# BaratiLab/MeshDQN

Measured on AMD Instinct MI355X. Metric: env steps/sec (ys930 ~2k-tri), higher is better.
Workload: dtype f64; 1 GPU; ys930 (876 vertices / 1570 triangles), 128 envs per GPU, S3 env step (remesh+smooth+interp+forces+state+1 IPCS step+Q-fwd); mesh=ys930, envs_per_gpu=128, parallelism=dp1 (independent envs sharded, no data-path collective)

## Files before the change

### meshdqn_amd/csrc/mdq_smooth_linear.hip

```cpp
#include <hip/hip_runtime.h>

#include <cstdlib>

#include "../../include/meshdqn_hip.h"
#include "mdq_internal.h"

namespace mdq_smooth_lin {
constexpr int LNV = 1024;
constexpr int LNT = 2048;
#ifndef MDQ_SMOOTH_LWG
#define MDQ_SMOOTH_LWG 768
#endif
constexpr int LWG = MDQ_SMOOTH_LWG;
constexpr int SCT = 512;
constexpr int TRW = LWG / 64 < 11 ? LWG / 64 : 11;
static_assert(LWG == 512 || LWG == 768, "workgroup shape");
constexpr int BS = 32;
constexpr int NSLOT = 14;
constexpr int NNARROW = 4;
constexpr int MAXNB = 16;
constexpr int MAXLOW = 8;
constexpr int SROW = 32;
constexpr int ZOFF = LNV * 16;
constexpr int PBUF = (LNV + 1) * 16;
// ... 274 lines not shown
  const double* mgs = reinterpret_cast<const double*>(mg);
  unsigned char* cur = lds + OFF_CUR;
  double* G = reinterpret_cast<double*>(lds + OFF_G);
  const int* ptr = reinterpret_cast<const int*>(lds + OFF_PTR);
  for (int b = 0; b < nb; ++b) {
    const u4 meta = *reinterpret_cast<const u4*>(lds + OFF_SROW + (b * BS + i) * SROW + h * 16);
    d2 M[8];
    load_m(M, mg, b, i, h);
    const d2 v0 = *reinterpret_cast<const d2*>(cur + (meta.x & 0xFFFF)), v1 = *reinterpret_cast<const d2*>(cur + (meta.x >> 16));
    const d2 v2 = *reinterpret_cast<const d2*>(cur + (meta.y & 0xFFFF)), v3 = *reinterpret_cast<const d2*>(cur + (meta.y >> 16));
    const d2 v4 = *reinterpret_cast<const d2*>(cur + (meta.z & 0xFFFF)), v5 = *reinterpret_cast<const d2*>(cur + (meta.z >> 16));
    const d2 v6 = *reinterpret_cast<const d2*>(cur + (meta.w & 0xFFFF));
    const double gx = halves_sum(((v0.x + v1.x) + (v2.x + v3.x)) + ((v4.x + v5.x) + v6.x));
    const double gy = halves_sum(((v0.y + v1.y) + (v2.y + v3.y)) + ((v4.y + v5.y) + v6.y));
    if (h == 0) {
      G[i] = gx;
      G[BS + i] = gy;
    }
    asm volatile("" ::: "memory");
    const d2* gqx = reinterpret_cast<const d2*>(G + 16 * h);
    const d2* gqy = reinterpret_cast<const d2*>(G + BS + 16 * h);
    double ax0 = 0.0, ax1 = 0.0, ay0 = 0.0, ay1 = 0.0;
#pragma unroll
    for (int t = 0; t < 8; ++t) {
      const d2 ggx = gqx[t], ggy = gqy[t];
      ax0 = __builtin_fma(M[t].x, ggx.x, ax0);
      ax1 = __builtin_fma(M[t].y, ggx.y, ax1);
      ay0 = __builtin_fma(M[t].x, ggy.x, ay0);
      ay1 = __builtin_fma(M[t].y, ggy.y, ay1);
    }
    const double xx = halves_sum(ax0 + ax1), xy = halves_sum(ay0 + ay1);
    const int soff = meta.w >> 16;
    if (h == 0) *reinterpret_cast<d2*>(cur + soff) = d2{xx, xy};
    asm volatile("" ::: "memory");
    unsigned long long fm = __builtin_amdgcn_ballot_w64(h == 0 && fixv[soff >> 4] != 0);
    while (fm) {
      const int r = __ffsll((long long)fm) - 1;
      fm &= fm - 1;
      const int v = __builtin_amdgcn_readlane(soff, r) >> 4;
      const d2 xs = exact_vertex(lds, v, l, OLD);
      const d2 xt = *reinterpret_cast<const d2*>(cur + v * 16);
      const double kk = (double)(ptr[v + 1] - ptr[v]);
      const double ddx = (xs.x - xt.x) * kk, ddy = (xs.y - xt.y) * kk;
      const double mjr = mgs[(((size_t)(b * 2 + (r >> 4)) * 8 + ((r & 15) >> 1)) * 32 + i) * 2 + (r & 1)];
      if (h == 0 && i >= r) {
        d2 xc = *reinterpret_cast<const d2*>(cur + soff);
        xc.x = __builtin_fma(mjr, ddx, xc.x);
        xc.y = __builtin_fma(mjr, ddy, xc.y);
        if (i == r) xc = xs;
        *reinterpret_cast<d2*>(cur + soff) = xc;
      }
      asm volatile("" ::: "memory");
    }
  }
}

__device__ __forceinline__ void sequential_sweep(unsigned char* lds, int n_int, int lane) {
  const uint16_t* ivert = reinterpret_cast<const uint16_t*>(lds + OFF_IVERT);
  unsigned char* cur = lds + OFF_CUR;
  for (int r = 0; r < n_int; ++r) {
    const int v = ivert[r];
    const d2 xs = exact_vertex(lds, v, lane & 7, cur);
    if (lane == 0) *reinterpret_cast<d2*>(cur + v * 16) = xs;
    asm volatile("" ::: "memory");
  }
}

#ifdef MDQ_LIN_TRACE
__device__ long long mdq_lin_trace_buf[16];
#define LT_STAMP(k) { __syncthreads(); const long long tn_ = __builtin_amdgcn_s_memtime(); if (threadIdx.x == 0 && blockIdx.x == 0) mdq_lin_trace_buf[k] += tn_ - tq_; tq_ = tn_; }
extern "C" int mdq_lin_trace_host(long long* out, int reset) {
  if (hipMemcpyFromSymbol(out, HIP_SYMBOL(mdq_lin_trace_buf), sizeof(long long) * 16) != hipSuccess) return -1;
  if (reset) { long long z[16] = {0}; if (hipMemcpyToSymbol(HIP_SYMBOL(mdq_lin_trace_buf), z, sizeof z) != hipSuccess) return -1; }
  return 0;
}
#else
#define LT_STAMP(k)
#endif

__global__ __launch_bounds__(LWG) void smooth_linear_kernel(int NV, int NT, double* coords, const int32_t* cells,
                                                            const int32_t* nv_, const int32_t* nt_, const int32_t* iters_,
                                                            const int32_t* rem, const int32_t* rstat, int iters_env,
                                                            double* mws, int64_t mstride, int32_t* redo, int32_t* stats,
                                                            int gather_all) {
  __shared__ __attribute__((aligned(16))) unsigned char lds[LDS_BYTES];
  const int b = blockIdx.x, tid = threadIdx.x, lane = tid & 63, wave = tid >> 6;
  const int S = iters_ ? iters_[b] : ((rem[b] >= 0 && rstat[b] == 0) ? iters_env : 0);
  if (S <= 0) {
    if (tid == 0) redo[b] = stats[3 * b] = stats[3 * b + 1] = stats[3 * b + 2] = 0;
    return;
  }
  const int nv = nv_[b], nt = nt_[b];
  double2* x = reinterpret_cast<double2*>(coords) + (int64_t)b * NV;
  const int32_t* tri = cells + (int64_t)b * NT * 3;
  int* ptr = reinterpret_cast<int*>(lds + OFF_PTR);
  uint32_t* inc = reinterpret_cast<uint32_t*>(lds + OFF_INC);
  uint16_t* rk = reinterpret_cast<uint16_t*>(lds + OFF_RK);
  uint16_t* ivert = reinterpret_cast<uint16_t*>(lds + OFF_IVERT);
  unsigned char* lmeta = lds + OFF_LMETA;
  uint16_t* kdeg = reinterpret_cast<uint16_t*>(lds + OFF_KDEG);
  int* misc = reinterpret_cast<int*>(lds + OFF_MISC);
  int* part = reinterpret_cast<int*>(lds + OFF_PART);
  uint32_t* tmp = reinterpret_cast<uint32_t*>(lds + OFF_TMP);
  uint16_t* nbl = reinterpret_cast<uint16_t*>(lds + OFF_NB);
  int* cnt = reinterpret_cast<int*>(lds + OFF_SROW + 3 * LNT * 4);
  static_assert(3 * LNT * 4 + LNV * 4 <= LNV * SROW, "cnt scratch");
#ifdef MDQ_LIN_TRACE
  long long tq_ = __builtin_amdgcn_s_memtime();
#endif
  for (int v = tid; v < LNV; v += LWG) cnt[v] = 0;
  if (tid < 4) misc[tid] = tid == 2 ? 1 : tid == 3 && gather_all ? -1 : 0;
  if (tid < 32) reinterpret_cast<double*>(lds + OFF_R2K)[tid] = tid ? 1.0 / (2.0 * tid) : 0.0;
  __syncthreads();
  for (int t = tid; t < nt; t += LWG)
    for (int k = 0; k < 3; ++k) atomicAdd(&cnt[tri[3 * t + k]], 1);
  __syncthreads();
  scan_inclusive(cnt, part);
  for (int v = tid; v < LNV; v += LWG) ptr[v + 1] = cnt[v];
  if (tid == 0) ptr[0] = 0;
  __syncthreads();
  for (int v = tid; v < LNV; v += LWG) cnt[v] = 0;
  __syncthreads();
  for (int t = tid; t < nt; t += LWG) {
    const int vs[3] = {tri[3 * t], tri[3 * t + 1], tri[3 * t + 2]};
    for (int k = 0; k < 3; ++k) {
      const int v = vs[k], a = vs[(k + 1) % 3], c = vs[(k + 2) % 3];
      const int q = ptr[v] + atomicAdd(&cnt[v], 1);
      tmp[q] = (uint32_t)a | ((uint32_t)c << 10) | ((uint32_t)t << 20);
    }
  }
  __syncthreads();
  LT_STAMP(0)
  for (int v = tid; v < LNV; v += LWG) {
    const int q0 = ptr[v], k = ptr[v + 1] - q0;
    bool interior = v < nv && k > 0 && k <= MAXNB;
    if (v < nv && k > MAXNB) misc[2] = 0;
    int nn = 0;
    if (interior) {
      if (k <= 8) {
        uint32_t ent[8];
#pragma unroll
        for (int j = 0; j < 8; ++j) ent[j] = j < k ? tmp[q0 + j] : 0xFFFFFFFFu;
#pragma unroll
        for (int e = 0; e < 8; ++e) {
          int rank = 0;
#pragma unroll
          for (int j = 0; j < 8; ++j) rank += ent[j] < ent[e];
          if (e < k) inc[q0 + rank] = ent[e];
        }
      } else {
        for (int e = 0; e < k; ++e) {
          const uint32_t my = tmp[q0 + e];
          int rank = 0;
          for (int j = 0; j < k; ++j) rank += (tmp[q0 + j] >> 20) < (my >> 20);
          inc[q0 + rank] = my;
        }
      }
      for (int e = 0; e < k; ++e) {
        const uint32_t w = inc[q0 + e];
        for (int s = 0; s < 2; ++s) {
          const uint32_t id = s ? (w >> 10) & 0x3FF : w & 0x3FF;
          int f = -1;
          for (int j = 0; j < nn; ++j)
            if ((nbl[v * MAXNB + j] & 0x3FF) == id) f = j;
          if (f >= 0) {
            nbl[v * MAXNB + f] += 1 << 10;
          } else if (nn < MAXNB) {
            nbl[v * MAXNB + nn++] = (uint16_t)(id | (1 << 10));
          } else {
            interior = false;
          }
        }
      }
      for (int j = 0; j < nn; ++j) interior = interior && (nbl[v * MAXNB + j] >> 10) == 2;
      interior = interior && nn == k;
    }
    cnt[v] = interior ? 1 : 0;
  }
  __syncthreads();
  LT_STAMP(1)
  scan_inclusive(cnt, part);
  const int n_int = cnt[LNV - 1];
  const int nb = (n_int + BS - 1) / BS;
  __syncthreads();
  for (int v = tid; v < LNV; v += LWG) {
    const bool interior = cnt[v] != (v ? cnt[v - 1] : 0);
    rk[v] = interior ? (uint16_t)(cnt[v] - 1) : (uint16_t)0xFFFF;
    if (interior) ivert[cnt[v] - 1] = (uint16_t)v;
  }
  __syncthreads();
  for (int v = tid; v < nv; v += LWG)
    if (rk[v] == 0xFFFF)
      for (int q = ptr[v]; q < ptr[v + 1]; ++q) inc[q] = 0xFFFFFFFFu;
  LT_STAMP(2)
  for (int r = tid; r < nb * BS; r += LWG) {
    uint16_t slots[16];
#pragma unroll
    for (int s = 0; s < 16; ++s) slots[s] = (uint16_t)ZOFF;
    int ns = 0, nl = 0, k = 1;
    if (r < n_int) {
      const int v = ivert[r], q0 = ptr[v];
      k = ptr[v + 1] - q0;
      for (int j = 0; j < k; ++j) {
        const int w = nbl[v * MAXNB + j] & 0x3FF;
        const int rw = rk[w];
        if (rw != 0xFFFF && w < v && (rw >> 5) == (r >> 5)) {
          if (nl < MAXLOW) lmeta[r * MAXLOW + nl] = (unsigned char)(rw & 31);
          ++nl;
        } else {
          if (ns < NSLOT) {
            const int pos = (ns & 1) * 8 + (ns >> 1);
#pragma unroll
            for (int s = 0; s < 16; ++s)
              if (s == pos) slots[s] = (uint16_t)(w * 16);
          }
          ++ns;
        }
      }
      if (ns > NSLOT || nl > MAXLOW) misc[2] = 0;
      if (ns > 2 * NNARROW) atomicOr(&misc[3], 1 << (r >> 5));
      slots[7] = (uint16_t)(v * 16);
      for (int q = q0; q < q0 + k; ++q) {
        const uint32_t w = inc[q];
        const int a = w & 0x3FF, c = (w >> 10) & 0x3FF;
        inc[q] = (w & 0xFFFFF) | ((uint32_t)v << 20) | ((uint32_t)(rk[a] != 0xFFFF && a < v) << 30) |
                 ((uint32_t)(rk[c] != 0xFFFF && c < v) << 31);
      }
    }
    kdeg[r] = (uint16_t)(k | (min(nl, MAXLOW) << 8));
    uint32_t wds[8];
#pragma unroll
    for (int s = 0; s < 8; ++s) wds[s] = (uint32_t)slots[2 * s] | ((uint32_t)slots[2 * s + 1] << 16);
    *reinterpret_cast<u4*>(lds + OFF_SROW + r * SROW) = u4{wds[0], wds[1], wds[2], wds[3]};
    *reinterpret_cast<u4*>(lds + OFF_SROW + r * SROW + 16) = u4{wds[4], wds[5], wds[6], wds[7]};
  }
  __syncthreads();
  LT_STAMP(3)
  const bool eligible = misc[2] != 0 && n_int > 0;
  if (!eligible) {
    static_assert(mdq_smoothing::LDS_BYTES <= LDS_BYTES && mdq_smoothing::SNV == LNV && mdq_smoothing::SNT == LNT, "hand-back in place");
    __syncthreads();
    mdq_smoothing::smooth_env(lds, b, NV, NT, coords, cells, nv_, nt_, S, nullptr);
    if (tid == 0) {
      redo[b] = S;
      stats[3 * b] = stats[3 * b + 1] = stats[3 * b + 2] = 0;
    }
    return;
  }
  double* mg = mws + (int64_t)b * mstride;
  {
    double* T = reinterpret_cast<double*>(lds + OFF_TRI) + wave * 528;
    const double* r2ktab = reinterpret_cast<const double*>(lds + OFF_R2K);
    for (int blk = wave < TRW ? wave : nb; blk < nb; blk += TRW) {
      const int r0 = blk * BS, j = lane & 31;
      const uint32_t kdv = kdeg[r0 + j];
      const uint2 lmv = *reinterpret_cast<const uint2*>(lmeta + (r0 + j) * MAXLOW);
      if (lane < 32) {
        for (int i = 0; i < BS; ++i) {
          const uint32_t kd = (uint32_t)__builtin_amdgcn_readlane((int)kdv, i);
          const uint32_t lo = (uint32_t)__builtin_amdgcn_readlane((int)lmv.x, i), hi = (uint32_t)__builtin_amdgcn_readlane((int)lmv.y, i);
          const int nl = kd >> 8;
          double val = 0.0;
          for (int t = 0; t < nl; ++t) {
            const int w = (int)(((t < 4 ? lo : hi) >> (8 * (t & 3))) & 0xFFu);
            if (j <= w) val += T[w * (w + 1) / 2 + j];
          }
          val = val * (2.0 * r2ktab[kd & 0xFF]) + (i == j ? 1.0 : 0.0);
          if (j <= i) T[i * (i + 1) / 2 + j] = val;
          asm volatile("" ::: "memory");
        }
      }
      asm volatile("s_waitcnt lgkmcnt(0)" ::: "memory");
      const int i = lane & 31, h = lane >> 5;
      d2* out = reinterpret_cast<d2*>(mg) + ((size_t)(blk * 2 + h) * 8) * 32 + i;
      d2* out01 = reinterpret_cast<d2*>(lds + OFF_M01) + ((blk * 2 + h) * 8) * 32 + i;
      for (int t = 0; t < 8; ++t) {
        const int j0 = 16 * h + 2 * t;
        const double m0 = j0 <= i ? T[i * (i + 1) / 2 + j0] * (2.0 * r2ktab[kdeg[r0 + j0] & 0xFF]) : 0.0;
        const double m1 = j0 + 1 <= i ? T[i * (i + 1) / 2 + j0 + 1] * (2.0 * r2ktab[kdeg[r0 + j0 + 1] & 0xFF]) : 0.0;
        out[t * 32] = d2{m0, m1};
        if (blk < 2) out01[t * 32] = d2{m0, m1};
      }
      asm volatile("s_waitcnt lgkmcnt(0)" ::: "memory");
    }
  }
  __threadfence_block();
  __syncthreads();
  LT_STAMP(4)
  for (int v = tid; v <= LNV; v += LWG) {
    d2 p = {0.0, 0.0};
    if (v < nv) {
      const double2 xv = x[v];
      p = d2{xv.x, xv.y};
    }
    *reinterpret_cast<d2*>(lds + OFF_CUR + v * 16) = p;
    *reinterpret_cast<d2*>(lds + OFF_SNAP + v * 16) = p;
    *reinterpret_cast<d2*>(lds + OFF_SNAP + PBUF + v * 16) = p;
  }
  __syncthreads();
  LT_STAMP(5)
  const d2* mgd = reinterpret_cast<const d2*>(mg);
  constexpr int NVAL = 2 * (LWG / 256);
  const int vw = (wave & 3) >= 2 ? 2 * (wave >> 2) + (wave & 1) : -1;
  const int ne = 3 * nt, npass = (ne + 63) / 64;
  unsigned char* fixv = lds + OFF_FIXV;
  auto copy_pos = [&](int dst_off, int src_off) {
    for (int v = tid; v < nv; v += LWG)
      *reinterpret_cast<d2*>(lds + dst_off + v * 16) = *reinterpret_cast<const d2*>(lds + src_off + v * 16);
  };
  auto solve_fast = [&]() {
    if (wave == 0) {
      __builtin_amdgcn_s_setprio(3);
      solve_sweep<0>(lds, mgd, nb, lane);
      __builtin_amdgcn_s_setprio(0);
    } else if (wave == 1) {
      __builtin_amdgcn_s_setprio(3);
      solve_sweep<1>(lds, mgd, nb, lane);
      __builtin_amdgcn_s_setprio(0);
    }
  };
  int s = 0, n_repaired = 0, n_rounds = 0, n_sentback = 0, n_seq = 0;
  bool checked = true, pending = false;
  while (true) {
    if (s >= S && !pending) break;
    if (checked) {
      const int snap = OFF_SNAP + (s & 1) * PBUF;
      for (int v = tid; v < LNV + 16; v += LWG) fixv[v] = 0;
      int rounds = 0, nflag = 0;
      while (true) {
        __syncthreads();
        if (nflag == 0) {
          solve_fast();
        } else if (wave == 0) {
          repair_sweep(lds, mgd, nb, lane, lds + snap);
        }
        if (tid == 0) misc[1] = 0;
        __syncthreads();
        bool bad = false;
        for (int p = wave; p < npass; p += LWG / 64) bad |= validate_entry<true>(lds, 64 * p + lane, ne, lds + snap, lds + OFF_CUR);
        if (bad) misc[1] = 1;
        __syncthreads();
        if (!misc[1]) break;
        nflag = 1;
        ++n_rounds;
        copy_pos(OFF_CUR, snap);
        if (++rounds >= MAXROUNDS) {
          __syncthreads();
          if (wave == 0) sequential_sweep(lds, n_int, lane);
          __syncthreads();
          ++n_seq;
          break;
        }
      }
      copy_pos(OFF_SNAP + ((s + 1) & 1) * PBUF, OFF_CUR);
      __syncthreads();
      ++s;
      if (rounds == 0) {
        checked = false;
        pending = false;
      } else {
        ++n_repaired;
      }
    } else {
      if (s < S) solve_fast();
      bool bad = false;
      if (pending) {
        const unsigned char* OLD = lds + OFF_SNAP + ((s - 1) & 1) * PBUF;
        const unsigned char* NEW = lds + OFF_SNAP + (s & 1) * PBUF;
        if (s < S) {
          if (vw >= 0)
            for (int p = vw; p < npass; p += NVAL) bad |= validate_entry<false>(lds, 64 * p + lane, ne, OLD, NEW);
        } else {
          for (int p = wave; p < npass; p += LWG / 64) bad |= validate_entry<false>(lds, 64 * p + lane, ne, OLD, NEW);
        }
      }
      if (tid == 0) misc[1] = 0;
      __syncthreads();
      if (bad) misc[1] = 1;
      __syncthreads();
      if (misc[1]) {
        --s;
        ++n_sentback;
        copy_pos(OFF_CUR, OFF_SNAP + (s & 1) * PBUF);
        checked = true;
        pending = false;
        __syncthreads();
        continue;
      }
      if (s >= S) break;
      copy_pos(OFF_SNAP + ((s + 1) & 1) * PBUF, OFF_CUR);
      __syncthreads();
      pending = true;
      ++s;
    }
  }
  LT_STAMP(6)
  __syncthreads();
  for (int v = tid; v < nv; v += LWG) {
    const d2 p = *reinterpret_cast<const d2*>(lds + OFF_CUR + v * 16);
    x[v] = double2{p.x, p.y};
  }
  if (tid == 0) {
    redo[b] = 0;
    stats[3 * b] = n_repaired;
    stats[3 * b + 1] = n_rounds;
    stats[3 * b + 2] = n_sentback | (n_seq << 16);
  }
}

__global__ void count_redo_kernel(int B, const int32_t* redo, unsigned long long* total) {
  const int b = blockIdx.x * blockDim.x + threadIdx.x;
  if (b < B && redo[b] > 0) atomicAdd(total, 1ull);
}
}

extern "C" int64_t mdq_smooth_fast_workspace_bytes(int32_t B, int32_t NV) {
  if (B <= 0 || NV <= 0) return 0;
  if (NV > mdq_smooth_lin::LNV)
    return smooth_big_workspace_bytes(B, NV, 1);
  const int64_t blocks = (NV + mdq_smooth_lin::BS - 1) / mdq_smooth_lin::BS + 2;
  return (int64_t)B * blocks * mdq_smooth_lin::MBLK * 8 + (int64_t)B * 16 + 256;
}

static int smooth_fast_impl(const char* who, int32_t B, int32_t NV, int32_t NT, double* coords, const int32_t* cells,
                            const int32_t* nv, const int32_t* nt, const int32_t* iterations, const int32_t* rem,
                            const int32_t* rstat, int32_t iters_env, void* workspace, int64_t workspace_bytes, void* stream) {
  if (B <= 0 || !coords || !cells || !nv || !nt || (!iterations && (!rem || !rstat)) || !workspace)
    return mdq_set_error("mdq_smooth_fast: bad arguments");
  if (NV > mdq_smooth_lin::LNV || NT > mdq_smooth_lin::LNT)
    return smooth_big_launch(B, NV, NT, coords, cells, nv, nt, iterations, rem, rstat, iters_env, workspace, workspace_bytes, stream);
  if (workspace_bytes < mdq_smooth_fast_workspace_bytes(B, NV) || (reinterpret_cast<uintptr_t>(workspace) & 15))
    return mdq_set_error("mdq_smooth_fast: workspace too small or not 16-byte aligned (mdq_smooth_fast_workspace_bytes)");
  (void)who;
  const int64_t blocks = (NV + mdq_smooth_lin::BS - 1) / mdq_smooth_lin::BS + 2;
  const int64_t mstride = blocks * mdq_smooth_lin::MBLK;
  double* mws = reinterpret_cast<double*>(workspace);
  int32_t* redo = reinterpret_cast<int32_t*>(mws + (int64_t)B * mstride);
  hipStream_t st = (hipStream_t)stream;
  static const int gather_all = [] {
    const char* e = std::getenv("MDQ_SMOOTH_GATHER");
    return e && std::atoi(e) == 7 ? 1 : 0;
  }();
  hipLaunchKernelGGL(mdq_smooth_lin::smooth_linear_kernel, dim3(B), dim3(mdq_smooth_lin::LWG), 0, st, NV, NT, coords, cells, nv,
                     nt, iterations, rem, rstat, iters_env, mws, mstride, redo, redo + B, gather_all);
  if (hipGetLastError() != hipSuccess) return mdq_set_error("mdq_smooth_fast: launch failed");
  return 0;
}

extern "C" int mdq_smooth_fast(int32_t B, int32_t NV, int32_t NT, double* coords, const int32_t* cells, const int32_t* nv,
                               const int32_t* nt, const int32_t* iterations, void* workspace, int64_t workspace_bytes,
                               void* stream) {
  if (!iterations) return mdq_set_error("mdq_smooth_fast: bad arguments");
  return smooth_fast_impl("mdq_smooth_fast", B, NV, NT, coords, cells, nv, nt, iterations, nullptr, nullptr, 0, workspace,
                          workspace_bytes, stream);
}

extern "C" int mdq_smooth_fast_env(int32_t B, int32_t NV, int32_t NT, double* coords, const int32_t* cells, const int32_t* nv,
                                   const int32_t* nt, const int32_t* rem, const int32_t* rstat, int32_t iterations,
                                   void* workspace, int64_t workspace_bytes, void* stream) {
  if (!rem || !rstat) return mdq_set_error("mdq_smooth_fast_env: bad arguments");
  return smooth_fast_impl("mdq_smooth_fast_env", B, NV, NT, coords, cells, nv, nt, nullptr, rem, rstat, iterations, workspace,
                          workspace_bytes, stream);
}
```

### meshdqn_amd/csrc/mdq_topology.hip

```cpp
#include <hip/hip_runtime.h>

#include <type_traits>

#include "../../include/meshdqn_hip.h"
#include "mdq_internal.h"

namespace mdq_topo {

#ifndef MDQ_TOPO_TW
#define MDQ_TOPO_TW 1024
#endif
constexpr int TW = MDQ_TOPO_TW;
template <int K>
struct TCap {
  static constexpr int NV = 1024 * K, NT = 2048 * K, NE = 3072 * K, NP = NV + NE, NS = 3 * NT, HS = 8192 * K;
  static constexpr int VBITS = K == 1 ? 10 : (K == 4 ? 12 : 14), HSHIFT = K == 1 ? 19 : (K == 4 ? 17 : 15), PER = NS / TW;
  using own_t = typename std::conditional<(K > 4), uint32_t, uint16_t>::type;
  static constexpr size_t BASE = ((size_t)16 * NV + 8 * HS + sizeof(int) * NS + sizeof(uint16_t) * NS + 2 * sizeof(uint16_t) * NE + sizeof(own_t) * NE +
                                  NE + NV + sizeof(int) * (TW + 16) + 15) & ~(size_t)15;
  using stage_t = typename std::conditional<(K > 4), uint32_t, uint16_t>::type;
  static constexpr size_t BYTES = BASE + (K > 4 ? sizeof(uint32_t) * 6 * NT : 0);
};
template <int PER>
struct Flags {
  uint32_t w[(PER + 31) / 32];
  __device__ __forceinline__ void set(int i, bool v) {
    if ((i & 31) == 0) w[i >> 5] = 0u;
    w[i >> 5] |= v ? 1u << (i & 31) : 0u;
  }
  __device__ __forceinline__ bool get(int i) const { return (w[i >> 5] >> (i & 31)) & 1u; }
};
constexpr int TNV = TCap<1>::NV, TNT = TCap<1>::NT, TNP = TCap<1>::NP;
constexpr uint32_t EMPTY = 0xFFFFFFFFu;
constexpr int TNPOLY = 256;

template <int PER>
__device__ __forceinline__ int scan_excl(int* a, int n, int* part) {
  const int tid = threadIdx.x;
  int run = 0, tid1 = tid;
  asm volatile("" : "+v"(tid1));
#pragma unroll
  for (int i = 0; i < PER; ++i) {
    const int idx = tid1 * PER + i;
    run += idx < n ? a[idx] : 0;
  }
  const int lane = tid & 63, wave = tid >> 6;
  int v = run;
#pragma unroll
  for (int off = 1; off < 64; off <<= 1) {
    const int u = __shfl_up(v, off, 64);
    if (lane >= off) v += u;
  }
  __syncthreads();
  if (lane == 63) part[wave] = v;
  __syncthreads();
  int pre = 0, total = 0;
#pragma unroll
  for (int w = 0; w < TW / 64; ++w) {
    const int wt = part[w];
    if (w < wave) pre += wt;
    total += wt;
  }
  int at = pre + v - run;
  int tid2 = tid;
  asm volatile("" : "+v"(tid2));
#pragma unroll
  for (int i = 0; i < PER; ++i) {
    const int idx = tid2 * PER + i;
    if (idx < n) {
      const int val = a[idx];
      a[idx] = at;
      at += val;
    }
  }
  __syncthreads();
  return total;
}

template <int SH>
__device__ __forceinline__ uint32_t hslot_t(uint32_t key) { return (key * 2654435761u) >> SH; }

__device__ __forceinline__ double seg_dist2(double px, double py, double ax, double ay, double bx, double by) {
#pragma clang fp contract(off)
  const double abx = bx - ax, aby = by - ay;
  double t = ((px - ax) * abx + (py - ay) * aby) / (abx * abx + aby * aby);
  t = t < 0.0 ? 0.0 : (t > 1.0 ? 1.0 : t);
  const double qx = ax + t * abx - px, qy = ay + t * aby - py;
  return qx * qx + qy * qy;
}

#ifdef MDQ_TOPO_TRACE
__device__ long long mdq_topo_trace_buf[16];
#define TT_STAMP(k) { const long long tn_ = __builtin_amdgcn_s_memtime(); if (threadIdx.x == 0 && blockIdx.x == 0) mdq_topo_trace_buf[k] += tn_ - tq_; tq_ = tn_; }
extern "C" int mdq_topo_trace_host(long long* out, int reset) {
  if (hipMemcpyFromSymbol(out, HIP_SYMBOL(mdq_topo_trace_buf), sizeof(long long) * 16) != hipSuccess) return -1;
  if (reset) { long long z[16] = {0}; if (hipMemcpyToSymbol(HIP_SYMBOL(mdq_topo_trace_buf), z, sizeof z) != hipSuccess) return -1; }
  return 0;
}
#else
#define TT_STAMP(k) { if (K != 1) asm volatile("" : "+v"(tid)); }
#endif

template <int K>
__global__ __launch_bounds__(TW) void topology_kernel(mdq_env_topo_desc D, mdq_ipcs_topo_out O, int has_ipcs,
                                                      int32_t* status, unsigned char* slab, mdq_topo_handover HO) {
#pragma clang fp contract(off)
#ifdef MDQ_TOPO_TRACE
  long long tq_ = __builtin_amdgcn_s_memtime();
#endif
  using CP = TCap<K>;
  constexpr int TNV = CP::NV, TNE = CP::NE, TNP = CP::NP, TNS = CP::NS, HSZ = CP::HS, PER = CP::PER;
  constexpr int TNT = CP::NT;
  (void)TNT;
  constexpr int TPOLY = K > 4 ? 512 : TNPOLY, NGMAX = TPOLY / 4;
  using cq_t = typename std::conditional<(K > 4), unsigned long long, uint32_t>::type;
  using fm_t = typename std::conditional<(K > 4), unsigned __int128, unsigned long long>::type;
  constexpr int CQB = K > 4 ? 16 : 8;
  constexpr int HT = K == 4 ? 16384 : HSZ;
  auto hslot = [](uint32_t key) { return hslot_t<(K == 4 ? 18 : CP::HSHIFT)>(key); };
  auto scan_excl = [](int* a_, int n_, int* part_) __attribute__((always_inline)) { return mdq_topo::scan_excl<CP::PER>(a_, n_, part_); };
  extern __shared__ __align__(16) unsigned char lds_[];
  unsigned char* smem = K == 1 ? lds_ : slab + (size_t)blockIdx.x * ((CP::BYTES + 255) & ~(size_t)255);
  double2* X = reinterpret_cast<double2*>(smem);
  uint32_t* hkey = K == 4 ? reinterpret_cast<uint32_t*>(lds_) : reinterpret_cast<uint32_t*>(smem + 16 * TNV);
  uint32_t* hval = hkey + HT;
  int* scanb = reinterpret_cast<int*>(smem + 16 * TNV + 8 * HSZ);
  uint16_t* eid_slot = reinterpret_cast<uint16_t*>(scanb + TNS);
  uint16_t* ea = eid_slot + TNS;
  uint16_t* eb = ea + TNE;
  using own_t = typename CP::own_t;
  own_t* eown = reinterpret_cast<own_t*>(eb + TNE);
  uint8_t* eflag = reinterpret_cast<uint8_t*>(eown + TNE);
  uint8_t* onb = eflag + TNE;
  int* part = reinterpret_cast<int*>(onb + TNV);
  int* misc = part + TW;
  unsigned char* R = smem + 16 * TNV;
  constexpr int RPOLY = 16 * TNV, RSEG = RPOLY + 16 * TPOLY;
  uint16_t* blist = reinterpret_cast<uint16_t*>(R);
  uint16_t* remv = blist + TNV;
  uint16_t* order = remv + TNV;
  int16_t* inv = reinterpret_cast<int16_t*>(order + TNV);
  double* dist = K == 4 ? reinterpret_cast<double*>(lds_ + 65536 + 28672) : reinterpret_cast<double*>(R + 8 * TNV);
  unsigned char* PB = K == 1 ? R + RPOLY : (K == 4 ? lds_ + 65536 : lds_);
  unsigned char* GB = K == 1 ? nullptr : (K == 4 ? lds_ + 65536 + 16384 : lds_ + 32768);
  double2* poly = reinterpret_cast<double2*>(PB);
  int* cntd = reinterpret_cast<int*>(R + RSEG);
  int* fill = cntd + TNP + 8;

  const int b = blockIdx.x;
  int tid = threadIdx.x;
  const int nv = D.nv[b], nt = D.nt[b];
  const int64_t Bq = b;
  const double* xg = D.coords + Bq * D.NV * 2;
  const int32_t* tri = D.cells + Bq * D.NT * 3;
  int32_t* cd = D.cell_dofs + Bq * 6 * D.NT;
  double* pts = D.points + Bq * D.NP * 2;
  if (tid == 0) status[b] = 0;
  int32_t* hcd = HO.cell_dofs ? HO.cell_dofs + Bq * 6 * D.NT : nullptr;
  for (int v = tid; v < TNV; v += TW) {
    if (v < nv) {
      X[v] = make_double2(xg[2 * v], xg[2 * v + 1]);
      if (HO.coords) reinterpret_cast<double2*>(HO.coords)[Bq * D.NV + v] = X[v];
    }
    onb[v] = 0;
  }
  if (HO.cells)
    for (int i = tid; i < 3 * nt; i += TW) HO.cells[Bq * D.NT * 3 + i] = tri[i];
  if (tid == 0) {
    if (HO.nv) HO.nv[b] = nv;
    if (HO.nt) HO.nt[b] = nt;
  }
  for (int h = tid; h < HT; h += TW) {
    hkey[h] = EMPTY;
    hval[h] = 0x7FFFFFFFu;
  }
  __syncthreads();

  TT_STAMP(0)
  auto slot_key = [&](int s, int& a, int& c) {
    const int t = s / 3, k = s - 3 * t;
    const int va = tri[3 * t + (k == 0 ? 1 : 0)], vb = tri[3 * t + (k == 2 ? 1 : 2)];
    a = min(va, vb);
    c = max(va, vb);
    return ((uint32_t)a << CP::VBITS) | (uint32_t)c;
  };
  auto probe = [&](uint32_t key) {
    uint32_t h = hslot(key);
    for (int n_ = 0; hkey[h] != key && n_ < HT; ++n_) h = (h + 1) & (HT - 1);
// ... 808 lines not shown
    const int f = idx / 18, rem = idx - 18 * f, q = rem / 6, j = rem - 6 * q;
    const int e = ofe[f];
    const int c = eown[e] / 3, k = eown[e] % 3;
    const int rowl = q == 0 ? (k == 0 ? 1 : 0) : (q == 1 ? (k == 2 ? 1 : 2) : 3 + k);
    const int row = cd[rowl * D.NT + c], col = cd[j * D.NT + c];
    ekey[idx] = ((EKey)row << RSH) | ((EKey)col << CSH);
    esrc[idx] = c * 36 + rowl * 6 + j;
  }
  __syncthreads();
  TT_STAMP(14)
  {
    int32_t* bo_rows = O.bo_rows + Bq * O.NBO;
    int32_t* bo_ptr = O.bo_ptr + Bq * (O.NBO + 1);
    int32_t* bo_col = O.bo_col + Bq * O.NBE;
    int32_t* bo_src = O.bo_src + Bq * O.NBE;
    int* lrow = reinterpret_cast<int*>(R + ROFE + 1024);
    {
      const int QE = (nent + 3) >> 2;
      for (int it0 = 0; it0 < 4 * nent; it0 += TW) {
        const int it = it0 + tid, t = min(it >> 2, nent - 1), part_ = it & 3;
        const EKey kt = ekey[t];
        const int st = esrc[t];
        const int q0 = part_ * QE, q1 = min(nent, q0 + QE);
        int rank = 0;
#pragma unroll 8
        for (int q = q0; q < q1; ++q) rank += (ekey[q] < kt) || (ekey[q] == kt && esrc[q] < st);
        rank += __shfl_xor(rank, 1, 64);
        rank += __shfl_xor(rank, 2, 64);
        if (part_ == 0 && (it >> 2) < nent) {
          bo_col[rank] = (int32_t)((kt >> CSH) & CMASK);
          bo_src[rank] = st;
          cntd[rank] = (int32_t)(kt >> RSH);
        }
      }
    }
    __syncthreads();
    TT_STAMP(15)
    for (int t = tid; t < TNS; t += TW) scanb[t] = (t < nent && (t == 0 || cntd[t] != cntd[t - 1])) ? 1 : 0;
    __syncthreads();
#pragma unroll
    for (int i = 0; i < PER; ++i) flg.set(i, scanb[tid * PER + i] != 0);
    __syncthreads();
    const int nbo = scan_excl(scanb, TNS, part);
    if (nbo > O.NBO) {
      if (tid == 0) status[b] = -5;
      return;
    }
#pragma unroll
    for (int i = 0; i < PER; ++i) {
      const int t = tid * PER + i;
      if (t < nent && flg.get(i)) {
        bo_rows[scanb[t]] = cntd[t];
        lrow[scanb[t]] = cntd[t];
        bo_ptr[scanb[t]] = t;
      }
    }
    if (tid == 0) {
      bo_ptr[nbo] = nent;
      O.nbo[b] = nbo;
      misc[0] = 0;
    }
    __syncthreads();
    for (int t = tid; t < (K == 1 ? nbo : 0); t += TW) {
      int same = 0;
      const int mine = lrow[t] % 512;
#pragma unroll 8
      for (int q = 0; q < nbo; ++q) same += (lrow[q] % 512) == mine;
      if (same > 2) misc[0] = 1;
    }
    __syncthreads();
    if (misc[0]) {
      if (tid == 0) status[b] = -4;
      return;
    }
  }
  TT_STAMP(8)
  if (K == 1)
    for (int i = 0; i < 6; ++i)
      for (int t = tid; t < nt; t += TW) scat[i * D.NT + t] = cd[i * D.NT + t] | (i == 0 ? ((int32_t)(cof[t] + 1) << 28) : 0);
  using stage_t = typename CP::stage_t;
  stage_t* stage = K > 4 ? reinterpret_cast<stage_t*>(smem + CP::BASE) : reinterpret_cast<stage_t*>(R);
  static_assert(K > 4 || 6 * TNT * 2 <= RSEG + (TNP + 8) * 4, "gather staging fits in front of `fill`");
  auto gather = [&](int nl, int ndof, int32_t* gptr, int32_t* gsrc) {
    for (int i = tid; i < TNS; i += TW) scanb[i] = 0;
    __syncthreads();
    for (int i = 0; i < nl; ++i)
      for (int t = tid; t < nt; t += TW) atomicAdd(&scanb[cd[i * D.NT + t]], 1);
    __syncthreads();
    const int tot = scan_excl(scanb, TNS, part);
    (void)tot;
    for (int i = tid; i <= ndof; i += TW) {
      gptr[i] = i < ndof ? scanb[i] : nl * nt;
      if (i < ndof) fill[i] = 0;
    }
    __syncthreads();
    for (int i = 0; i < nl; ++i)
      for (int t = tid; t < nt; t += TW) {
        const int dof = cd[i * D.NT + t];
        stage[scanb[dof] + atomicAdd(&fill[dof], 1)] = (stage_t)(t * nl + i);
      }
    __syncthreads();
    for (int i = tid; i < ndof; i += TW) {
      const int q0 = scanb[i], q1 = q0 + fill[i];
      for (int a_ = q0 + 1; a_ < q1; ++a_) {
        const stage_t w = stage[a_];
        int j = a_ - 1;
        while (j >= q0 && stage[j] > w) {
          stage[j + 1] = stage[j];
          --j;
        }
        stage[j + 1] = w;
      }
    }
    __syncthreads();
    for (int q = tid; q < nl * nt; q += TW) gsrc[q] = stage[q];
    if (nl == 6) {
      int32_t* g1p_ = O.g1_ptr + Bq * (D.NV + 1);
      int32_t* g1s_ = O.g1_src + Bq * 3 * D.NT;
      for (int i = tid; i <= nv; i += TW) g1p_[i] = i < nv ? scanb[i] : 3 * nt;
      for (int q = tid; q < 3 * nt; q += TW) {
        const int w = stage[q];
        g1s_[q] = (w / 6) * 3 + (w - (w / 6) * 6);
      }
    }
    __syncthreads();
  };
  TT_STAMP(9)
  TT_STAMP(10)
  gather(6, n2, O.g2_ptr + Bq * (D.NP + 1), O.g2_src + Bq * 6 * D.NT);
  TT_STAMP(11)
  uint16_t* adjl = reinterpret_cast<uint16_t*>(R);
  int* rptr = cntd;
  int* rcur = cntd + TNV + 8;
  for (int i = tid; i < TNS; i += TW) scanb[i] = 0;
  __syncthreads();
  for (int e = tid; e < ne; e += TW) {
    atomicAdd(&scanb[ea[e]], 1);
    atomicAdd(&scanb[eb[e]], 1);
  }
  __syncthreads();
  for (int i = tid; i < nv; i += TW) {
    fill[i] = scanb[i] + 1;
    rcur[i] = 0;
  }
  __syncthreads();
  scan_excl(scanb, TNS, part);
  for (int i = tid; i <= nv; i += TW) rptr[i] = i < nv ? scanb[i] : 2 * ne;
  __syncthreads();
  for (int e = tid; e < ne; e += TW) {
    const int a_ = ea[e], b_ = eb[e];
    adjl[rptr[a_] + atomicAdd(&rcur[a_], 1)] = (uint16_t)b_;
    adjl[rptr[b_] + atomicAdd(&rcur[b_], 1)] = (uint16_t)a_;
  }
  __syncthreads();
  {
    int32_t* so = O.sl1_off + Bq * (D.NV / 64 + 2);
    int32_t* sc = O.sl1_col + Bq * O.NSE1;
    const int ns = (nv + 63) / 64;
    for (int s_ = tid; s_ < TNS; s_ += TW) scanb[s_] = 0;
    __syncthreads();
    for (int s_ = tid >> 6; s_ < ns; s_ += TW / 64) {
      const int r = 64 * s_ + (tid & 63);
      int w = r < nv ? fill[r] : 0;
#pragma unroll
      for (int o = 32; o > 0; o >>= 1) w = max(w, __shfl_xor(w, o, 64));
      if ((tid & 63) == 0) scanb[s_] = 64 * w;
    }
    __syncthreads();
    const int total = scan_excl(scanb, TNS, part);
    if (total > O.NSE1) {
      if (tid == 0) status[b] = -6;
      return;
    }
    for (int s_ = tid; s_ <= ns; s_ += TW) so[s_] = s_ < ns ? scanb[s_] : total;
    for (int r = tid; r < 64 * ns; r += TW) {
      const int s_ = r >> 6, l = r & 63;
      const int base = scanb[s_], w = ((s_ + 1 < ns ? scanb[s_ + 1] : total) - base) >> 6;
      const int rr = min(r, nv - 1);
      int len = 0;
      if (r < nv) {
        const int q0 = rptr[r], q1 = rptr[r + 1];
        len = q1 - q0 + 1;
        int below = 0;
        for (int q = q0; q < q1; ++q) {
          const int v = adjl[q];
          int rank = v > r ? 1 : 0;
          for (int q2 = q0; q2 < q1; ++q2) rank += adjl[q2] < v ? 1 : 0;
          below += v < r ? 1 : 0;
          sc[base + 64 * rank + l] = v;
        }
        sc[base + 64 * below + l] = r;
      }
      for (int j = len; j < w; ++j) sc[base + 64 * j + l] = rr;
    }
  }
  TT_STAMP(6)
}

}

extern "C" int64_t mdq_env_topology_workspace_bytes(const mdq_env_topo_desc* d) {
  if (!d || d->B <= 0) return 0;
  if (d->NV <= mdq_topo::TNV && d->NT <= mdq_topo::TNT && d->NP <= mdq_topo::TNP) return 0;
  using C4 = mdq_topo::TCap<4>;
  using C16 = mdq_topo::TCap<16>;
  if (d->NV > C16::NV || d->NT > C16::NT || d->NP > C16::NP) return -1;
  if (d->NV > C4::NV || d->NT > C4::NT || d->NP > C4::NP) return (int64_t)((C16::BYTES + 255) & ~(size_t)255) * d->B;
  return (int64_t)((C4::BYTES + 255) & ~(size_t)255) * d->B;
}

extern "C" int mdq_env_topology(const mdq_env_topo_desc* d, void* stream, int32_t* status) {
  if (!d || d->B <= 0 || !status) return mdq_set_error("mdq_env_topology: bad arguments");
  if ((d->poly_ptr == nullptr) != (d->src_of_env == nullptr))
    return mdq_set_error("mdq_env_topology: poly_ptr and src_of_env go together");
  {
    using C4_ = mdq_topo::TCap<4>;
    const bool huge_ = d->NV > C4_::NV || d->NT > C4_::NT || d->NP > C4_::NP;
    if (d->npoly > (huge_ ? 2 : 1) * mdq_topo::TNPOLY)
      return mdq_set_error("mdq_env_topology: more than 256 polygon points (512 for the 16384-vertex instance)");
  }
  mdq_ipcs_topo_out o = {};
  if (d->ipcs) o = *d->ipcs;
  mdq_topo_handover h = {};
  if (d->handover) h = *d->handover;
  if (d->NV <= mdq_topo::TNV && d->NT <= mdq_topo::TNT && d->NP <= mdq_topo::TNP) {
    const size_t lds = mdq_topo::TCap<1>::BYTES;
    static const hipError_t attr = hipFuncSetAttribute(reinterpret_cast<const void*>(&mdq_topo::topology_kernel<1>),
                                                       hipFuncAttributeMaxDynamicSharedMemorySize, 160 * 1024);
    if (attr != hipSuccess) return mdq_set_error("hipFuncSetAttribute(topology_kernel) failed");
    hipLaunchKernelGGL(mdq_topo::topology_kernel<1>, dim3(d->B), dim3(mdq_topo::TW), lds, (hipStream_t)stream, *d, o,
                       d->ipcs ? 1 : 0, status, nullptr, h);
  } else {
    using C4 = mdq_topo::TCap<4>;
    using C16 = mdq_topo::TCap<16>;
    if (d->NV > C16::NV || d->NT > C16::NT || d->NP > C16::NP)
      return mdq_set_error("mdq_env_topology: capacity above 16384 vertices / 32768 triangles / 65536 P2 dofs");
    const bool huge = d->NV > C4::NV || d->NT > C4::NT || d->NP > C4::NP;
    if (!d->workspace || d->workspace_bytes < mdq_env_topology_workspace_bytes(d) || (reinterpret_cast<uintptr_t>(d->workspace) & 15))
      return mdq_set_error("mdq_env_topology: workspace missing, too small or not 16-byte aligned (mdq_env_topology_workspace_bytes)");
    unsigned char* slab = static_cast<unsigned char*>(d->workspace);
    const size_t lds4 = 2 * sizeof(uint32_t) * 16384;
    static const hipError_t attr4 = hipFuncSetAttribute(reinterpret_cast<const void*>(&mdq_topo::topology_kernel<4>),
                                                        hipFuncAttributeMaxDynamicSharedMemorySize, (int)lds4);
    if (attr4 != hipSuccess) return mdq_set_error("hipFuncSetAttribute(topology_kernel<4>) failed");
    if (huge) {
      static const hipError_t attr16 = hipFuncSetAttribute(reinterpret_cast<const void*>(&mdq_topo::topology_kernel<16>),
                                                           hipFuncAttributeMaxDynamicSharedMemorySize, (int)lds4);
      if (attr16 != hipSuccess) return mdq_set_error("hipFuncSetAttribute(topology_kernel<16>) failed");
      hipLaunchKernelGGL(mdq_topo::topology_kernel<16>, dim3(d->B), dim3(mdq_topo::TW), lds4, (hipStream_t)stream, *d, o,
                         d->ipcs ? 1 : 0, status, slab, h);
    } else
    hipLaunchKernelGGL(mdq_topo::topology_kernel<4>, dim3(d->B), dim3(mdq_topo::TW), lds4, (hipStream_t)stream, *d, o,
                       d->ipcs ? 1 : 0, status, slab, h);
  }
  if (hipGetLastError() != hipSuccess) return mdq_set_error("topology_kernel launch failed");
  return 0;
}
```

Before: 181,800 env steps/s.

## Streamline smoothing and topology setup with register sorts and skipped inverse rows

The smoothing setup now builds each vertex's neighbour list from a fixed 16-entry register dedup, replacing the serial LDS search. The block-inverse factor loop visits only rows that have lower neighbours, using a ballot mask, and reads precomputed column factors from scratch. The topology kernel fills P2 edge dofs directly from the edge ownership tables instead of running atomics, and ranks short lists with branch-free 8-wide sorts. All new paths are on by default, with environment flags to restore the old ones. The cost is extra register pressure and assumptions about small vertex degree.

New measurement: 184,800 env steps/s, median of 6. 1.7% higher.

```diff
diff --git a/meshdqn_amd/csrc/mdq_smooth_linear.hip b/meshdqn_amd/csrc/mdq_smooth_linear.hip
--- a/meshdqn_amd/csrc/mdq_smooth_linear.hip
+++ b/meshdqn_amd/csrc/mdq_smooth_linear.hip
@@ -380,9 +380,10 @@
                                                             const int32_t* nv_, const int32_t* nt_, const int32_t* iters_,
                                                             const int32_t* rem, const int32_t* rstat, int iters_env,
                                                             double* mws, int64_t mstride, int32_t* redo, int32_t* stats,
-                                                            int gather_all) {
+                                                            int flags) {
   __shared__ __attribute__((aligned(16))) unsigned char lds[LDS_BYTES];
   const int b = blockIdx.x, tid = threadIdx.x, lane = tid & 63, wave = tid >> 6;
+  const bool gather_all = flags & 1, nb_loop = flags & 2, inv_all = flags & 4;
   const int S = iters_ ? iters_[b] : ((rem[b] >= 0 && rstat[b] == 0) ? iters_env : 0);
   if (S <= 0) {
     if (tid == 0) redo[b] = stats[3 * b] = stats[3 * b + 1] = stats[3 * b + 2] = 0;
@@ -435,6 +436,7 @@
     if (v < nv && k > MAXNB) misc[2] = 0;
     int nn = 0;
     if (interior) {
+      bool listed = false;
       if (k <= 8) {
         uint32_t ent[8];
 #pragma unroll
@@ -445,6 +447,28 @@
 #pragma unroll
           for (int j = 0; j < 8; ++j) rank += ent[j] < ent[e];
           if (e < k) inc[q0 + rank] = ent[e];
+        }
+        if (!nb_loop) {
+          static_assert(OFF_INC + (3 * LNT + 8) * 4 <= LDS_BYTES, "batched read of the sorted cells");
+          asm volatile("" ::: "memory");
+          uint32_t ids[16];
+#pragma unroll
+          for (int e = 0; e < 8; ++e) {
+            const uint32_t w = inc[q0 + e];
+            ids[2 * e] = e < k ? w & 0x3FF : 0x400u + 2 * e;
+            ids[2 * e + 1] = e < k ? (w >> 10) & 0x3FF : 0x401u + 2 * e;
+          }
+          bool third = false;
+#pragma unroll
+          for (int p = 0; p < 16; ++p) {
+            int seen = 0;
+#pragma unroll
+            for (int q = 0; q < p; ++q) seen += ids[q] == ids[p];
+            third = third | (seen > 1);
+            if (p < 2 * k && seen == 0) nbl[v * MAXNB + nn++] = (uint16_t)ids[p];
+          }
+          interior = !third && nn == k;
+          listed = true;
         }
       } else {
         for (int e = 0; e < k; ++e) {
@@ -454,24 +478,26 @@
           inc[q0 + rank] = my;
         }
       }
-      for (int e = 0; e < k; ++e) {
-        const uint32_t w = inc[q0 + e];
-        for (int s = 0; s < 2; ++s) {
-          const uint32_t id = s ? (w >> 10) & 0x3FF : w & 0x3FF;
-          int f = -1;
-          for (int j = 0; j < nn; ++j)
-            if ((nbl[v * MAXNB + j] & 0x3FF) == id) f = j;
-          if (f >= 0) {
-            nbl[v * MAXNB + f] += 1 << 10;
-          } else if (nn < MAXNB) {
-            nbl[v * MAXNB + nn++] = (uint16_t)(id | (1 << 10));
-          } else {
-            interior = false;
+      if (!listed) {
+        for (int e = 0; e < k; ++e) {
+          const uint32_t w = inc[q0 + e];
+          for (int s = 0; s < 2; ++s) {
+            const uint32_t id = s ? (w >> 10) & 0x3FF : w & 0x3FF;
+            int f = -1;
+            for (int j = 0; j < nn; ++j)
+              if ((nbl[v * MAXNB + j] & 0x3FF) == id) f = j;
+            if (f >= 0) {
+              nbl[v * MAXNB + f] += 1 << 10;
+            } else if (nn < MAXNB) {
+              nbl[v * MAXNB + nn++] = (uint16_t)(id | (1 << 10));
+            } else {
+              interior = false;
+            }
           }
         }
-      }
-      for (int j = 0; j < nn; ++j) interior = interior && (nbl[v * MAXNB + j] >> 10) == 2;
-      interior = interior && nn == k;
+        for (int j = 0; j < nn; ++j) interior = interior && (nbl[v * MAXNB + j] >> 10) == 2;
+        interior = interior && nn == k;
+      }
     }
     cnt[v] = interior ? 1 : 0;
   }
@@ -553,33 +579,81 @@
       const int r0 = blk * BS, j = lane & 31;
       const uint32_t kdv = kdeg[r0 + j];
       const uint2 lmv = *reinterpret_cast<const uint2*>(lmeta + (r0 + j) * MAXLOW);
-      if (lane < 32) {
-        for (int i = 0; i < BS; ++i) {
-          const uint32_t kd = (uint32_t)__builtin_amdgcn_readlane((int)kdv, i);
-          const uint32_t lo = (uint32_t)__builtin_amdgcn_readlane((int)lmv.x, i), hi = (uint32_t)__builtin_amdgcn_readlane((int)lmv.y, i);
-          const int nl = kd >> 8;
-          double val = 0.0;
-          for (int t = 0; t < nl; ++t) {
-            const int w = (int)(((t < 4 ? lo : hi) >> (8 * (t & 3))) & 0xFFu);
-            if (j <= w) val += T[w * (w + 1) / 2 + j];
+      if (inv_all) {
+        if (lane < 32) {
+          for (int i = 0; i < BS; ++i) {
+            const uint32_t kd = (uint32_t)__builtin_amdgcn_readlane((int)kdv, i);
+            const uint32_t lo = (uint32_t)__builtin_amdgcn_readlane((int)lmv.x, i), hi = (uint32_t)__builtin_amdgcn_readlane((int)lmv.y, i);
+            const int nl = kd >> 8;
+            double val = 0.0;
+            for (int t = 0; t < nl; ++t) {
+              const int w = (int)(((t < 4 ? lo : hi) >> (8 * (t & 3))) & 0xFFu);
+              if (j <= w) val += T[w * (w + 1) / 2 + j];
+            }
+            val = val * (2.0 * r2ktab[kd & 0xFF]) + (i == j ? 1.0 : 0.0);
+            if (j <= i) T[i * (i + 1) / 2 + j] = val;
+            asm volatile("" ::: "memory");
           }
-          val = val * (2.0 * r2ktab[kd & 0xFF]) + (i == j ? 1.0 : 0.0);
-          if (j <= i) T[i * (i + 1) / 2 + j] = val;
-          asm volatile("" ::: "memory");
-        }
-      }
-      asm volatile("s_waitcnt lgkmcnt(0)" ::: "memory");
-      const int i = lane & 31, h = lane >> 5;
-      d2* out = reinterpret_cast<d2*>(mg) + ((size_t)(blk * 2 + h) * 8) * 32 + i;
-      d2* out01 = reinterpret_cast<d2*>(lds + OFF_M01) + ((blk * 2 + h) * 8) * 32 + i;
-      for (int t = 0; t < 8; ++t) {
-        const int j0 = 16 * h + 2 * t;
-        const double m0 = j0 <= i ? T[i * (i + 1) / 2 + j0] * (2.0 * r2ktab[kdeg[r0 + j0] & 0xFF]) : 0.0;
-        const double m1 = j0 + 1 <= i ? T[i * (i + 1) / 2 + j0 + 1] * (2.0 * r2ktab[kdeg[r0 + j0 + 1] & 0xFF]) : 0.0;
-        out[t * 32] = d2{m0, m1};
-        if (blk < 2) out01[t * 32] = d2{m0, m1};
-      }
-      asm volatile("s_waitcnt lgkmcnt(0)" ::: "memory");
+        }
+        asm volatile("s_waitcnt lgkmcnt(0)" ::: "memory");
+        const int i = lane & 31, h = lane >> 5;
+        d2* out = reinterpret_cast<d2*>(mg) + ((size_t)(blk * 2 + h) * 8) * 32 + i;
+        d2* out01 = reinterpret_cast<d2*>(lds + OFF_M01) + ((blk * 2 + h) * 8) * 32 + i;
+        for (int t = 0; t < 8; ++t) {
+          const int j0 = 16 * h + 2 * t;
+          const double m0 = j0 <= i ? T[i * (i + 1) / 2 + j0] * (2.0 * r2ktab[kdeg[r0 + j0] & 0xFF]) : 0.0;
+          const double m1 = j0 + 1 <= i ? T[i * (i + 1) / 2 + j0 + 1] * (2.0 * r2ktab[kdeg[r0 + j0 + 1] & 0xFF]) : 0.0;
+          out[t * 32] = d2{m0, m1};
+          if (blk < 2) out01[t * 32] = d2{m0, m1};
+        }
+        asm volatile("s_waitcnt lgkmcnt(0)" ::: "memory");
+      } else {
+        static_assert(TRW * BS * 8 <= LWG * 4, "column factors in the scan scratch");
+        double* ck = reinterpret_cast<double*>(lds + OFF_PART) + wave * BS;
+        const double rkv = 2.0 * r2ktab[kdv & 0xFF];
+        for (int q = lane; q < 528; q += 64) T[q] = 0.0;
+        if (lane < 32) {
+          T[j * (j + 3) / 2] = 1.0;
+          ck[j] = rkv;
+        }
+        uint32_t todo = (uint32_t)__builtin_amdgcn_ballot_w64(lane < 32 && (kdv >> 8) != 0);
+        const int rklo = __double2loint(rkv), rkhi = __double2hiint(rkv);
+        asm volatile("" ::: "memory");
+        if (lane < 32) {
+          while (todo) {
+            const int i = __builtin_ctz(todo);
+            todo &= todo - 1;
+            const uint32_t kd = (uint32_t)__builtin_amdgcn_readlane((int)kdv, i);
+            const uint32_t lo = (uint32_t)__builtin_amdgcn_readlane((int)lmv.x, i), hi = (uint32_t)__builtin_amdgcn_readlane((int)lmv.y, i);
+            const double rk = __hiloint2double(__builtin_amdgcn_readlane(rkhi, i), __builtin_amdgcn_readlane(rklo, i));
+            const int nl = kd >> 8;
+            double val = 0.0;
+            for (int t = 0; t < nl; ++t) {
+              const int w = (int)(((t < 4 ? lo : hi) >> (8 * (t & 3))) & 0xFFu);
+              if (j <= w) val += T[w * (w + 1) / 2 + j];
+            }
+            val = val * rk + (i == j ? 1.0 : 0.0);
+            if (j <= i) T[i * (i + 1) / 2 + j] = val;
+            asm volatile("" ::: "memory");
+          }
+        }
+        asm volatile("s_waitcnt lgkmcnt(0)" ::: "memory");
+        const int i = lane & 31, h = lane >> 5;
+        d2* out = reinterpret_cast<d2*>(mg) + ((size_t)(blk * 2 + h) * 8) * 32 + i;
+        d2* out01 = reinterpret_cast<d2*>(lds + OFF_M01) + ((blk * 2 + h) * 8) * 32 + i;
+        const double* row = T + i * (i + 1) / 2 + 16 * h;
+        const d2* cf = reinterpret_cast<const d2*>(ck + 16 * h);
+#pragma unroll
+        for (int t = 0; t < 8; ++t) {
+          const int j0 = 16 * h + 2 * t;
+          const double a0 = row[2 * t], a1 = row[2 * t + 1];
+          const d2 c = cf[t];
+          const double m0 = j0 <= i ? a0 * c.x : 0.0, m1 = j0 + 1 <= i ? a1 * c.y : 0.0;
+          out[t * 32] = d2{m0, m1};
+          if (blk < 2) out01[t * 32] = d2{m0, m1};
+        }
+        asm volatile("s_waitcnt lgkmcnt(0)" ::: "memory");
+      }
     }
   }
   __threadfence_block();
@@ -739,8 +813,12 @@
     const char* e = std::getenv("MDQ_SMOOTH_GATHER");
     return e && std::atoi(e) == 7 ? 1 : 0;
   }();
+  static const int setup_parent = [] {
+    const char* e = std::getenv("MDQ_SMOOTH_SETUP_PARENT");
+    return e ? std::atoi(e) & 3 : 0;
+  }();
   hipLaunchKernelGGL(mdq_smooth_lin::smooth_linear_kernel, dim3(B), dim3(mdq_smooth_lin::LWG), 0, st, NV, NT, coords, cells, nv,
-                     nt, iterations, rem, rstat, iters_env, mws, mstride, redo, redo + B, gather_all);
+                     nt, iterations, rem, rstat, iters_env, mws, mstride, redo, redo + B, gather_all | (setup_parent << 1));
   if (hipGetLastError() != hipSuccess) return mdq_set_error("mdq_smooth_fast: launch failed");
   return 0;
 }
diff --git a/meshdqn_amd/csrc/mdq_topology.hip b/meshdqn_amd/csrc/mdq_topology.hip
--- a/meshdqn_amd/csrc/mdq_topology.hip
+++ b/meshdqn_amd/csrc/mdq_topology.hip
@@ -1,5 +1,6 @@
 #include <hip/hip_runtime.h>
 
+#include <cstdlib>
 #include <type_traits>
 
 #include "../../include/meshdqn_hip.h"
@@ -103,7 +104,8 @@
 
 template <int K>
 __global__ __launch_bounds__(TW) void topology_kernel(mdq_env_topo_desc D, mdq_ipcs_topo_out O, int has_ipcs,
-                                                      int32_t* status, unsigned char* slab, mdq_topo_handover HO) {
+                                                      int32_t* status, unsigned char* slab, mdq_topo_handover HO,
+                                                      int idx_parent) {
 #pragma clang fp contract(off)
 #ifdef MDQ_TOPO_TRACE
   long long tq_ = __builtin_amdgcn_s_memtime();
@@ -1078,10 +1080,14 @@
   stage_t* stage = K > 4 ? reinterpret_cast<stage_t*>(smem + CP::BASE) : reinterpret_cast<stage_t*>(R);
   static_assert(K > 4 || 6 * TNT * 2 <= RSEG + (TNP + 8) * 4, "gather staging fits in front of `fill`");
   auto gather = [&](int nl, int ndof, int32_t* gptr, int32_t* gsrc) {
+    const bool direct = K == 1 && nl == 6 && !(idx_parent & 1);
+    const int nlv = direct ? 3 : nl;
     for (int i = tid; i < TNS; i += TW) scanb[i] = 0;
     __syncthreads();
-    for (int i = 0; i < nl; ++i)
+    for (int i = 0; i < nlv; ++i)
       for (int t = tid; t < nt; t += TW) atomicAdd(&scanb[cd[i * D.NT + t]], 1);
+    if (direct)
+      for (int e = tid; e < ne; e += TW) scanb[nv + e] = 2 - (eflag[e] & 1);
     __syncthreads();
     const int tot = scan_excl(scanb, TNS, part);
     (void)tot;
@@ -1090,14 +1096,32 @@
       if (i < ndof) fill[i] = 0;
     }
     __syncthreads();
-    for (int i = 0; i < nl; ++i)
+    for (int i = 0; i < nlv; ++i)
       for (int t = tid; t < nt; t += TW) {
         const int dof = cd[i * D.NT + t];
         stage[scanb[dof] + atomicAdd(&fill[dof], 1)] = (stage_t)(t * nl + i);
       }
-    __syncthreads();
-    for (int i = tid; i < ndof; i += TW) {
+    if (direct)
+      for (int s = tid; s < 3 * nt; s += TW) {
+        const int e = eid_slot[s], t = s / 3;
+        stage[scanb[nv + e] + (s != (int)eown[e] ? 1 : 0)] = (stage_t)(t * 6 + 3 + (s - 3 * t));
+      }
+    __syncthreads();
+    for (int i = tid; i < (direct ? nv : ndof); i += TW) {
       const int q0 = scanb[i], q1 = q0 + fill[i];
+      if (direct && q1 - q0 <= 8) {
+        uint32_t ent[8];
+#pragma unroll
+        for (int j = 0; j < 8; ++j) ent[j] = q0 + j < q1 ? (uint32_t)stage[q0 + j] : 0xFFFFFFFFu;
+#pragma unroll
+        for (int e = 0; e < 8; ++e) {
+          int rank = 0;
+#pragma unroll
+          for (int j = 0; j < 8; ++j) rank += ent[j] < ent[e];
+          if (q0 + e < q1) stage[q0 + rank] = (stage_t)ent[e];
+        }
+        continue;
+      }
       for (int a_ = q0 + 1; a_ < q1; ++a_) {
         const stage_t w = stage[a_];
         int j = a_ - 1;
@@ -1178,6 +1202,19 @@
         const int q0 = rptr[r], q1 = rptr[r + 1];
         len = q1 - q0 + 1;
         int below = 0;
+        if (K == 1 && !(idx_parent & 2) && q1 - q0 <= 8) {
+          uint32_t a[8];
+#pragma unroll
+          for (int j = 0; j < 8; ++j) a[j] = q0 + j < q1 ? (uint32_t)adjl[q0 + j] : 0xFFFFFFFFu;
+#pragma unroll
+          for (int e = 0; e < 8; ++e) {
+            int rank = a[e] > (uint32_t)r ? 1 : 0;
+#pragma unroll
+            for (int j = 0; j < 8; ++j) rank += a[j] < a[e];
+            below += a[e] < (uint32_t)r ? 1 : 0;
+            if (q0 + e < q1) sc[base + 64 * rank + l] = (int)a[e];
+          }
+        } else
         for (int q = q0; q < q1; ++q) {
           const int v = adjl[q];
           int rank = v > r ? 1 : 0;
@@ -1215,6 +1252,10 @@
     if (d->npoly > (huge_ ? 2 : 1) * mdq_topo::TNPOLY)
       return mdq_set_error("mdq_env_topology: more than 256 polygon points (512 for the 16384-vertex instance)");
   }
+  static const int idx_parent = [] {
+    const char* e = std::getenv("MDQ_TOPO_INDEX_PARENT");
+    return e ? std::atoi(e) & 3 : 0;
+  }();
   mdq_ipcs_topo_out o = {};
   if (d->ipcs) o = *d->ipcs;
   mdq_topo_handover h = {};
@@ -1225,7 +1266,7 @@
                                                        hipFuncAttributeMaxDynamicSharedMemorySize, 160 * 1024);
     if (attr != hipSuccess) return mdq_set_error("hipFuncSetAttribute(topology_kernel) failed");
     hipLaunchKernelGGL(mdq_topo::topology_kernel<1>, dim3(d->B), dim3(mdq_topo::TW), lds, (hipStream_t)stream, *d, o,
-                       d->ipcs ? 1 : 0, status, nullptr, h);
+                       d->ipcs ? 1 : 0, status, nullptr, h, idx_parent);
   } else {
     using C4 = mdq_topo::TCap<4>;
     using C16 = mdq_topo::TCap<16>;
@@ -1244,10 +1285,10 @@
                                                            hipFuncAttributeMaxDynamicSharedMemorySize, (int)lds4);
       if (attr16 != hipSuccess) return mdq_set_error("hipFuncSetAttribute(topology_kernel<16>) failed");
       hipLaunchKernelGGL(mdq_topo::topology_kernel<16>, dim3(d->B), dim3(mdq_topo::TW), lds4, (hipStream_t)stream, *d, o,
-                         d->ipcs ? 1 : 0, status, slab, h);
+                         d->ipcs ? 1 : 0, status, slab, h, idx_parent);
     } else
     hipLaunchKernelGGL(mdq_topo::topology_kernel<4>, dim3(d->B), dim3(mdq_topo::TW), lds4, (hipStream_t)stream, *d, o,
-                       d->ipcs ? 1 : 0, status, slab, h);
+                       d->ipcs ? 1 : 0, status, slab, h, idx_parent);
   }
   if (hipGetLastError() != hipSuccess) return mdq_set_error("topology_kernel launch failed");
   return 0;
```
